# Total-RD/pymgrid

Measured on AMD Instinct MI355X. Metric: microgrid env-steps/sec, higher is better.
Workload: dtype f64

## Files before the change

### include/mgx.h

```cpp
#ifndef MGX_H
#define MGX_H

#include <stddef.h>
#include <stdint.h>

#ifdef __cplusplus
extern "C" {
#endif

#define MGX_ABI_VERSION 9
#define MGX_ABI_MINOR 3

enum mgx_status {
    MGX_OK = 0,
    MGX_ERR_INVALID = 1,
    MGX_ERR_UNSUPPORTED = 2,
    MGX_ERR_RANGE = 3,
    MGX_ERR_DEVICE = 4
};

enum mgx_obs_format { MGX_OBS_F64 = 0, MGX_OBS_F32 = 1 };
enum mgx_action_format { MGX_ACT_F64 = 0, MGX_ACT_F32 = 1 };
enum mgx_obs_rows { MGX_OBS_ROWS_FULL = 0, MGX_OBS_ROWS_STATE_ONLY = 1, MGX_OBS_ROWS_STATE_COMPACT = 2 };
enum mgx_done_format { MGX_DONE_U8 = 0, MGX_DONE_BITS = 1 };
// ... 56 lines not shown
    const uint32_t *gen_times;
    const double *grid_max_import, *grid_max_export, *grid_cost_per_unit_co2;
    const double *loss_load_cost, *overgeneration_cost;
    const double *load_ts, *pv_ts, *grid_ts;
    const double *load_lo, *load_hi, *pv_lo, *pv_hi;
    const double *grid_lo, *grid_hi;
    const double *load_noise_std, *pv_noise_std, *grid_noise_std;
    double *charge, *soc;
    uint32_t *gen_status;
    const double *base_load, *base_pv, *base_co2;
    const uint8_t *load_profile, *pv_profile, *co2_profile, *tariff;
    const double *load_ratio, *pv_ratio;
    const uint64_t *outage_bits;
} mgx_columns;

#define MGX_PROFILE_PITCH 8

int mgx_abi_version(void);
int mgx_abi_minor(void);

enum mgx_tunable {
    MGX_TUNE_WIN_THREADS = 0,
    MGX_TUNE_WIN_GROUP = 1,
    MGX_TUNE_WIN_PAIRS = 2,
    MGX_TUNE_WIN_MIN_LDS = 3,
    MGX_TUNE_PREFETCH_POOL = 4,
    MGX_TUNE_MULTI_GENERIC = 5,
    MGX_TUNE_MULTI_SMALL_OWN = 6,
    MGX_TUNE_GRID_MAJOR_COPY = 7,
    MGX_TUNE_FLEET_BYVALUE = 8,
    MGX_TUNE_LAUNCH_THREADS = 9,
    MGX_TUNE_MULTI_STATIC = 10,
    MGX_TUNE_FLEET_EPISODES = 11,
    MGX_TUNE_COUNT_ = 12
};
int mgx_set_tunable(int32_t id, int64_t value);
int mgx_get_tunable(int32_t id, int64_t *value, int64_t *default_value);
const char *mgx_last_error(void);

int mgx_create(const mgx_layout *layout, const mgx_columns *columns, mgx_handle **out);
void mgx_destroy(mgx_handle *h);

int32_t mgx_action_dim(const mgx_handle *h);
int32_t mgx_obs_dim(const mgx_handle *h);
int32_t mgx_log_dim(const mgx_handle *h);
const char *mgx_log_name(const mgx_handle *h, int32_t column);
int32_t mgx_current_step(const mgx_handle *h);

int mgx_use_device_counter(mgx_handle *h, int enable, mgx_stream stream);

int mgx_reset(mgx_handle *h, int32_t initial_step, void *obs, mgx_stream stream);

int mgx_set_window(mgx_handle *h, int32_t initial_step, int32_t final_step);

int mgx_reset_windows(mgx_handle *h, const int32_t *start, const int32_t *length, int32_t max_length,
                      double *load_w, double *pv_w, double *grid_w, int32_t *final_rel, void *obs, mgx_stream stream);

int mgx_reset_windows_rolling(mgx_handle *h, const int32_t *start, const int32_t *length, int32_t max_length,
                              int32_t ring_rows, double *load_w, double *pv_w, double *grid_w, int32_t *final_abs, void *obs,
                              mgx_stream stream);
int mgx_reset_grids(mgx_handle *h, const uint8_t *mask, const int32_t *start, const int32_t *length, mgx_stream stream);
int mgx_reset_grids_random(mgx_handle *h, const uint8_t *mask, uint64_t seed, int32_t fixed_length, int32_t *start_io,
                           int32_t *length_io, int32_t *t0_io, mgx_stream stream);

int mgx_reset_episodes(mgx_handle *h, const int32_t *start, const int32_t *length, int32_t max_length, int32_t *row_off,
                       int32_t *final_abs, void *obs, mgx_stream stream);
int mgx_set_auto_reset(mgx_handle *h, int32_t enable, uint64_t seed, int32_t fixed_length, int32_t *start_io, int32_t *length_io,
// ... 111 lines not shown

int mgx_step_many(mgx_handle *h, const void *actions, int32_t K, int normalized,
                  double *reward, uint8_t *done, void *obs, double *log, mgx_stream stream);

typedef struct mgx_env_slot {
    double *reward;
    uint8_t *done;
    void *obs;
    double *log;
} mgx_env_slot;
#define MGX_ENV_MAX_SLOTS 128
typedef struct mgx_env_plan {
    int32_t struct_size;
    int32_t n_slots;
    const mgx_env_slot *slots;
    int32_t ring_K;
    int32_t n_actions;
    void *rings[3];
    const int32_t *table;
} mgx_env_plan;
int mgx_env_bind(mgx_handle *h, const mgx_env_plan *plan);
int mgx_env_seek(mgx_handle *h, int32_t next_slot, int32_t ring_idx, int32_t ring_pos);
int mgx_env_position(const mgx_handle *h, int32_t *last_slot, int32_t *ring_idx, int32_t *ring_pos);
int mgx_env_step(mgx_handle *h, const void *actions, int normalized, mgx_stream stream);
int mgx_env_step_discrete(mgx_handle *h, const int32_t *action_id, mgx_stream stream);

int mgx_action_bounds(mgx_handle *h, double *lo, double *hi, mgx_stream stream);

int mgx_set_shards(mgx_handle *h, int32_t n_shards);
int mgx_set_launch_threads(mgx_handle *h, int32_t mode);
int mgx_fork(mgx_handle *h, mgx_stream stream);
int mgx_join(mgx_handle *h, mgx_stream stream);
void *mgx_shard_stream(mgx_handle *h, int32_t shard);

typedef struct mgx_fleet_item {
    int32_t struct_size;
    int32_t n_actions;
    mgx_handle *handle;
    const void *actions;
    const int32_t *action_id;
    const int32_t *table;
    double *reward;
    uint8_t *done;
    void *obs;
    double *log;
    void *refill_ring;
    int32_t refill_K;
    int32_t refill_ahead;
    int32_t refill_chunk;
    int32_t refill_chunks;
    int32_t wait_prefetch;
    int32_t reserved;
} mgx_fleet_item;
int mgx_fleet_step(const mgx_fleet_item *items, int32_t n_items, int normalized, mgx_stream stream);
int mgx_fleet_env_step(mgx_handle *const *handles, const void *const *actions, int32_t n_handles, int normalized, mgx_stream stream);

typedef struct mgx_synth {
    int32_t struct_size;
    int32_t n_grids, n_steps;
    int32_t n_load_profiles, n_pv_profiles, n_co2_profiles;
    const double *base_load, *base_pv, *base_co2;
    const int32_t *load_profile, *pv_profile, *co2_profile;
    const double *load_ratio, *pv_ratio;
    const int32_t *tariff;
    const int32_t *weak;
    const double *outage_per_day;
// ... 47 lines not shown
```

### pymgrid_amd/_lib.py

```python
import ctypes as C
import json
import os
import re
import subprocess
import sys

_PKG = os.path.dirname(os.path.abspath(__file__))
_ROOT = os.path.dirname(_PKG)
LIB_PATH = os.environ.get("MGX_LIB") or os.path.join(_PKG, "libmgx.so")
UNITS = (
    ("mgx_abi.hip", None, 1),
    ("mgx_fused.hip", "MGX_FUSED_PART", 6),
    ("mgx_episodes.hip", "MGX_EPISODE_PART", 2),
    ("mgx_step_episodes.hip", "MGX_EPISODE_PART", 2),
    ("mgx_episode_rows.hip", "MGX_EPISODE_PART", 2),
    ("mgx_step_episode_rows.hip", "MGX_EPISODE_PART", 2),
    ("mgx_policy_episodes.hip", "MGX_EPISODE_PART", 2),
    ("mgx_step_policy_episodes.hip", "MGX_EPISODE_PART", 2),
)
SOURCES = [os.path.join(_PKG, "csrc", f) for f in [u[0] for u in UNITS] + ["mgx_kernels.hpp", "mgx_core.hpp", "mgx_episode_loop.hpp", "mgx_episode_rows.hpp", "mgx_policy.hpp"]] + \
          [os.path.join(_ROOT, "include", "mgx.h")]

HIPCC_FLAGS = ["--offload-arch=gfx950", "-O3", "-std=c++17", "-ffp-contract=off", "-fno-fast-math", "-fPIC"]

# ... 167 lines not shown
                                       C.c_void_p, C.c_void_p, C.POINTER(EpisodeStats), C.c_void_p]),
    "mgx_step_k_episodes": (C.c_int, [C.c_void_p, C.c_void_p, C.c_int32, C.c_int, C.c_void_p, C.c_void_p, C.c_void_p, C.c_void_p,
                                      C.POINTER(EpisodeStats), C.c_void_p]),
    "mgx_rollout_episodes_rows": (C.c_int, [C.c_void_p, C.c_void_p, C.c_int, c_i32_p, C.c_int32, C.c_int32, C.c_void_p, C.c_void_p,
                                            C.c_void_p, C.c_void_p, C.POINTER(EpisodeStats), C.POINTER(EpisodeRows), C.c_void_p]),
    "mgx_step_k_episodes_rows": (C.c_int, [C.c_void_p, C.c_void_p, C.c_int32, C.c_int, C.c_void_p, C.c_void_p, C.c_void_p, C.c_void_p,
                                           C.POINTER(EpisodeStats), C.POINTER(EpisodeRows), C.c_void_p]),
    "mgx_rollout_policy_episodes": (C.c_int, [C.c_void_p, C.POINTER(Policy), c_i32_p, C.c_int32, C.c_int32, C.c_void_p, C.c_void_p,
                                              C.c_void_p, C.c_void_p, C.c_void_p, C.POINTER(EpisodeStats), C.POINTER(EpisodeRows),
                                              C.c_void_p]),
    "mgx_step_k_policy_episodes": (C.c_int, [C.c_void_p, C.POINTER(Policy), C.c_int32, C.c_void_p, C.c_void_p, C.c_void_p, C.c_void_p,
                                             C.c_void_p, C.POINTER(EpisodeStats), C.POINTER(EpisodeRows), C.c_void_p]),
    "mgx_metrics": (C.c_int, [C.c_void_p, C.c_void_p, C.c_int32, C.c_void_p, C.c_void_p]),
    "mgx_reset_windows": (C.c_int, [C.c_void_p, C.c_void_p, C.c_void_p, C.c_int32, C.c_void_p, C.c_void_p, C.c_void_p,
                                    C.c_void_p, C.c_void_p, C.c_void_p]),
    "mgx_reset_windows_rolling": (C.c_int, [C.c_void_p, C.c_void_p, C.c_void_p, C.c_int32, C.c_int32] + [C.c_void_p] * 6),
    "mgx_reset_grids": (C.c_int, [C.c_void_p, C.c_void_p, C.c_void_p, C.c_void_p, C.c_void_p]),
    "mgx_reset_grids_random": (C.c_int, [C.c_void_p, C.c_void_p, C.c_uint64, C.c_int32, C.c_void_p, C.c_void_p, C.c_void_p, C.c_void_p]),
    "mgx_reset_episodes": (C.c_int, [C.c_void_p, C.c_void_p, C.c_void_p, C.c_int32] + [C.c_void_p] * 4),
    "mgx_set_auto_reset": (C.c_int, [C.c_void_p, C.c_int32, C.c_uint64, C.c_int32, C.c_void_p, C.c_void_p, C.c_void_p]),
    "mgx_set_final_obs": (C.c_int, [C.c_void_p, C.c_void_p]),
    "mgx_check_step": (C.c_int, [C.c_void_p, C.c_void_p, C.c_int, C.c_void_p, C.c_void_p]),
    "mgx_step_many": (C.c_int, [C.c_void_p, C.c_void_p, C.c_int32, C.c_int, C.c_void_p, C.c_void_p, C.c_void_p, C.c_void_p,
                                C.c_void_p]),
    "mgx_env_bind": (C.c_int, [C.c_void_p, C.POINTER(EnvPlan)]),
    "mgx_env_seek": (C.c_int, [C.c_void_p, C.c_int32, C.c_int32, C.c_int32]),
    "mgx_env_position": (C.c_int, [C.c_void_p, c_i32_p, c_i32_p, c_i32_p]),
    "mgx_env_step": (C.c_int, [C.c_void_p, C.c_void_p, C.c_int, C.c_void_p]),
    "mgx_env_step_discrete": (C.c_int, [C.c_void_p, C.c_void_p, C.c_void_p]),
    "mgx_set_shards": (C.c_int, [C.c_void_p, C.c_int32]),
    "mgx_fork": (C.c_int, [C.c_void_p, C.c_void_p]),
    "mgx_join": (C.c_int, [C.c_void_p, C.c_void_p]),
    "mgx_shard_stream": (C.c_void_p, [C.c_void_p, C.c_int32]),
    "mgx_fleet_step": (C.c_int, [C.POINTER(FleetItem), C.c_int32, C.c_int, C.c_void_p]),
    "mgx_fleet_env_step": (C.c_int, [C.POINTER(C.c_void_p), C.POINTER(C.c_void_p), C.c_int32, C.c_int, C.c_void_p]),
    "mgx_synthesize_series": (C.c_int, [C.POINTER(Synth), C.c_void_p]),
    "mgx_generate_columns": (C.c_int, [C.POINTER(Gen), C.c_void_p]),
}


def source_hash(extra=()):
    import hashlib
    h = hashlib.sha256()
    for f in sorted(SOURCES):
        h.update(os.path.basename(f).encode() + b"\0")
        with open(f, "rb") as fh:
            h.update(fh.read())
    h.update(" ".join(HIPCC_FLAGS + list(extra)).encode())
    return h.hexdigest()[:16]


def built_hash(lib_path=None):
    try:
        with open((lib_path or LIB_PATH) + ".srchash") as fh:
            return fh.read().strip() or None
    except OSError:
        return None


def up_to_date(lib_path=None):
    path = lib_path or LIB_PATH
    return os.path.exists(path) and built_hash(path) == source_hash()


def build(force=False, verbose=False, defs=(), lib_path=None, abi_only=False):
    if lib_path is not None or defs:
# ... 94 lines not shown
    f = os.path.join(_PKG, "csrc", "_build", "resource_usage.json")
    try:
        with open(f) as fh:
            return json.load(fh)
    except (OSError, ValueError):
        return None


_lib = None


def lib():
    global _lib
    if _lib is None:
        if not os.path.exists(LIB_PATH):
            raise ImportError(f"{LIB_PATH} is missing: build it with __graft_entry__.build() "
                              f"(pymgrid_amd has no CPU fallback)")
        L = C.CDLL(LIB_PATH)
        for name, (res, args) in SYMBOLS.items():
            fn = getattr(L, name)
            fn.restype, fn.argtypes = res, args
        if L.mgx_abi_version() != ABI_VERSION:
            raise ImportError(f"libmgx.so ABI {L.mgx_abi_version()} != binding ABI {ABI_VERSION}; rebuild")
        assert C.sizeof(Layout) == 64
        _lib = L
    return _lib


def check(rc):
    if rc != MGX_OK:
        raise MgxError(rc, lib().mgx_last_error().decode())


def set_tunable(name, value):
    check(lib().mgx_set_tunable(TUNABLES.index(name), int(value)))


def get_tunable(name):
    v, d = C.c_int64(), C.c_int64()
    check(lib().mgx_get_tunable(TUNABLES.index(name), C.byref(v), C.byref(d)))
    return v.value, d.value
```

### pymgrid_amd/csrc/mgx_abi.hip

```cpp
#include "mgx_kernels.hpp"
#include "mgx_episode_rows.hpp"
#include "mgx_policy.hpp"

#include <cstdarg>
#include <cstdio>
#include <cstdlib>
#include <cstring>
#include <atomic>
#include <chrono>
#include <condition_variable>
#include <mutex>
#include <new>
#include <string>
#include <thread>
#include <vector>

using namespace mgx;

#define MGX_MAX_SHARDS 8

struct mgx_handle {
    KArgs k;
    mgx_layout layout;
    int32_t window_lo, window_hi;
    bool multi;
    int32_t ring_pitch;
    size_t multi_lds;
    int multi_small;
    std::vector<std::string> log_names;
    int32_t *d_lists;
    std::vector<int32_t> lists_uploaded;
    int32_t *d_counter;
    int32_t n_cu;
    int32_t flags;
    int32_t t;
    int32_t action_dim;
    int device;
    double *scratch;
    int32_t n_shards;
    int32_t shard_lo[MGX_MAX_SHARDS + 1];
    hipStream_t shard_stream[MGX_MAX_SHARDS];
    hipEvent_t shard_event[MGX_MAX_SHARDS];
    hipEvent_t fork_event;
    int32_t launch_threads;
    hipStream_t counter_stream;
    KArgs *d_kargs;
    KArgs k_uploaded;
    bool k_uploaded_valid;
    PLWords *d_table;
    PLWords table_uploaded;
    bool table_uploaded_valid;
    bool env_bound;
    int32_t env_n_slots, env_next, env_ring_K, env_ring_idx, env_ring_pos, env_n_actions;
    mgx_env_slot env_slots[MGX_ENV_MAX_SLOTS];
    char *env_rings[3];
    int32_t env_table[12 * 3 * 2];
    hipStream_t prefetch_stream;
    bool prefetch_pooled;
    hipEvent_t prefetch_gate, prefetch_done;
    bool prefetch_pending;
    bool windowed;
    bool rolling;
    bool inplace;
    double *pm_tables;
    double *gm_tables;
    int32_t gm_pitch;
    int32_t pm_pitch;
    int32_t rolling_max_length;
    double *roll_load_w, *roll_pv_w, *roll_grid_w;
    int32_t *roll_final;
    const double *full_load_ts, *full_pv_ts, *full_grid_ts;
    mgx_columns full_c;
    int32_t full_T, full_final, full_initial, full_window_lo, full_window_hi;
};

namespace {

constexpr int MAX_PARTIAL = 1024;
constexpr int MAX_METRICS = 64;

thread_local char g_err[512] = "";

constexpr int MGX_MAX_DEVICES = 16;
hipStream_t g_shard_streams[MGX_MAX_DEVICES][MGX_MAX_SHARDS] = {};
std::mutex g_shard_streams_lock;
hipStream_t g_prefetch_streams[MGX_MAX_DEVICES] = {};

std::atomic<int64_t> g_tune[MGX_TUNE_COUNT_];
const int64_t kTuneDefault[MGX_TUNE_COUNT_] = {
     0,
     0,
     -1,
     -1,
     0,
     0,
     1,
     1,
     1,
     1,
     1,
     1,
};
struct TuneInit { TuneInit() { for (int j = 0; j < MGX_TUNE_COUNT_; j++) g_tune[j].store(kTuneDefault[j], std::memory_order_relaxed); } } g_tune_init;
inline int64_t tune(int id) { return g_tune[id].load(std::memory_order_relaxed); }

struct LaunchWorker {
    std::atomic<uint64_t> posted{0}, done{0};
    std::atomic<int> asleep{0};
    void (*fn)(void *, int) = nullptr;
    void *ctx = nullptr;
    int shard = 0, device = 0;
    hipError_t err = hipSuccess;
    std::mutex sleep_lock, caller_lock;
    std::condition_variable wake;
    std::thread th;
    static constexpr int SPIN_US = 500;

    void run()
    {
        (void)hipSetDevice(device);
        uint64_t seen = 0;
        for (;;) {
            auto idle_since = std::chrono::steady_clock::now();
            unsigned spins = 0;
            while (posted.load(std::memory_order_acquire) == seen) {
                __builtin_ia32_pause();
                if ((++spins & 1023) == 0 &&
                    std::chrono::steady_clock::now() - idle_since > std::chrono::microseconds(SPIN_US)) {
                    std::unique_lock<std::mutex> lk(sleep_lock);
                    asleep.store(1, std::memory_order_seq_cst);
                    wake.wait(lk, [&] { return posted.load(std::memory_order_seq_cst) != seen; });
                    asleep.store(0, std::memory_order_seq_cst);
                }
            }
// ... 172 lines not shown
        case 5: { constexpr int F = 5; CALL; } break;   \
        case 6: { constexpr int F = 6; CALL; } break;   \
        case 7: { constexpr int F = 7; CALL; } break;   \
        case 14: { constexpr int F = 14; CALL; } break; \
        default: { constexpr int F = 15; CALL; } break; \
    }

}

static int32_t fused_grids_per_block(const mgx_handle *h, int64_t N)
{
    const int cus = h->n_cu > 0 ? h->n_cu : 256;
    int32_t best = BLOCK_K;
    int64_t best_cost = -1;
    for (int32_t g = BLOCK_K; g >= BLOCK_K * 3 / 4; g -= 16) {
        const int64_t blocks = (N + g - 1) / g;
        const int64_t cost = ((blocks + cus - 1) / cus) * g;
        if (best_cost < 0 || cost < best_cost) { best_cost = cost; best = g; }
    }
    return best;
}

static FusedLaunch fused_launch_for(const mgx_handle *h, const KArgs &k, hipStream_t s, const FusedOut &fo, int32_t K)
{
    FusedLaunch L;
    L.flags = h->flags; L.act_f32 = false; L.rich = fo.log != nullptr || fo.status_trace != nullptr; L.fact = factorised(k.c); L.per_step = false;
    L.gpb = fused_grids_per_block(h, k.g1 - k.g0);
    L.blocks = (unsigned)((k.g1 - k.g0 + L.gpb - 1) / L.gpb);
    L.stream = s; L.k = &k; L.actions = nullptr; L.tab = nullptr; L.ids = nullptr;
    L.t = t_arg(h); L.K = K; L.normalized = 0; L.out = fo;
    return L;
}

template <int F, bool NOISE, typename OT>
static void launch_obs_rows_as(const KArgs &k, const WindowPlan &plan, int32_t t, void *obs, unsigned blocks, size_t lds, hipStream_t st)
{
    if (lds > 64 * 1024)
        (void)hipFuncSetAttribute((const void *)obs_rows_wave_kernel<F, NOISE, OT>, hipFuncAttributeMaxDynamicSharedMemorySize, (int)lds);
    obs_rows_wave_kernel<F, NOISE, OT><<<blocks, 64, lds, st>>>(k, plan, t, (OT *)obs);
}

template <int F>
static void launch_obs_rows(const KArgs &k, const WindowPlan &plan, int32_t t, void *obs, unsigned blocks, size_t lds,
                            hipStream_t st)
{
    if (noisy(k.c)) {
        if (k.obs_f32) launch_obs_rows_as<F, true, float>(k, plan, t, obs, blocks, lds, st);
        else launch_obs_rows_as<F, true, double>(k, plan, t, obs, blocks, lds, st);
    } else {
        if (k.obs_f32) launch_obs_rows_as<F, false, float>(k, plan, t, obs, blocks, lds, st);
        else launch_obs_rows_as<F, false, double>(k, plan, t, obs, blocks, lds, st);
    }
}

static void opt_in_160k_lds(const void *kernel, bool *opted_in)
{
    int dev = 0;
    (void)hipGetDevice(&dev);
    if (dev < 0 || dev >= MGX_MAX_DEVICES || !opted_in[dev]) {
        (void)hipFuncSetAttribute(kernel, hipFuncAttributeMaxDynamicSharedMemorySize, 160 * 1024);
        if (dev >= 0 && dev < MGX_MAX_DEVICES) opted_in[dev] = true;
    }
}

template <int F, typename OT>
static void launch_windows_kernel(const KArgs &k, const WindowsKPlan &plan, int32_t t, void *ring, unsigned blocks, size_t lds, hipStream_t st)
// ... 28 lines not shown
        return MGX_OK;
    }
    const int32_t D = h->k.obs_dim;
    WindowPlan plan;
    plan.grid_col_base = h->k.col_grid;
    plan.ld = D | 1;
    plan.group = 16;
    const size_t esz = h->k.obs_f32 ? sizeof(float) : sizeof(double);
    while (plan.group > 1 && (size_t)plan.group * plan.ld * esz > 160 * 1024) plan.group /= 2;
    const size_t lds = ((size_t)plan.group * plan.ld * esz + 7) & ~(size_t)7;
    if (lds > 160 * 1024)
        return fail(MGX_ERR_UNSUPPORTED, "observation rows of %d values do not fit the 160 KiB LDS tile (horizon too large)", D);
    const unsigned blocks = (unsigned)(((int64_t)h->k.N + plan.group - 1) / plan.group);
    MGX_DISPATCH_F(h->flags, (launch_obs_rows<F>(h->k, plan, t, obs, blocks, lds, st)));
    return MGX_OK;
}

extern "C" {

int mgx_abi_version(void) { return MGX_ABI_VERSION; }
int mgx_abi_minor(void) { return MGX_ABI_MINOR; }

int mgx_set_tunable(int32_t id, int64_t value)
{
    g_err[0] = 0;
    if (id < 0 || id >= MGX_TUNE_COUNT_) return fail(MGX_ERR_INVALID, "mgx_set_tunable: unknown tunable %d", id);
    bool ok = true;
    switch (id) {
        case MGX_TUNE_WIN_THREADS: ok = value == 0 || value == 256 || value == 512 || value == 1024; break;
        case MGX_TUNE_WIN_GROUP: ok = value >= 0 && value <= 64; break;
        case MGX_TUNE_WIN_PAIRS: ok = value >= -1 && value <= 1; break;
        case MGX_TUNE_WIN_MIN_LDS: ok = value >= -1 && value <= 160 * 1024; break;
        case MGX_TUNE_LAUNCH_THREADS: ok = value >= 0 && value <= 2; break;
        default: ok = value == 0 || value == 1; break;
    }
    if (!ok) return fail(MGX_ERR_INVALID, "mgx_set_tunable: value %lld is not valid for tunable %d", (long long)value, id);
    g_tune[id].store(value, std::memory_order_relaxed);
    return MGX_OK;
}

int mgx_get_tunable(int32_t id, int64_t *value, int64_t *default_value)
{
    g_err[0] = 0;
    if (id < 0 || id >= MGX_TUNE_COUNT_) return fail(MGX_ERR_INVALID, "mgx_get_tunable: unknown tunable %d", id);
    if (value) *value = tune(id);
    if (default_value) *default_value = kTuneDefault[id];
    return MGX_OK;
}

int mgx_set_launch_threads(mgx_handle *h, int32_t enable)
{
    g_err[0] = 0;
    if (!h) return fail(MGX_ERR_INVALID, "mgx_set_launch_threads: NULL handle");
    if (enable < 0 || enable > 2) return fail(MGX_ERR_INVALID, "mgx_set_launch_threads: mode must be 0, 1 or 2");
    h->launch_threads = enable;
    return MGX_OK;
}

const char *mgx_last_error(void) { return g_err; }

int mgx_create(const mgx_layout *L, const mgx_columns *C, mgx_handle **out)
{
    g_err[0] = 0;
    if (!L || !C || !out) return fail(MGX_ERR_INVALID, "mgx_create: NULL argument");
    *out = nullptr;
    if (L->struct_size != (int32_t)sizeof(mgx_layout) || C->struct_size != (int32_t)sizeof(mgx_columns))
// ... 108 lines not shown
    h->d_kargs = nullptr; h->k_uploaded_valid = false;
    h->d_table = nullptr; h->table_uploaded_valid = false;
    h->env_bound = false; h->env_n_slots = 0; h->env_next = 0; h->env_ring_K = 0; h->env_ring_idx = 0; h->env_ring_pos = 0; h->env_n_actions = 0;
    h->prefetch_stream = nullptr; h->prefetch_gate = nullptr; h->prefetch_done = nullptr; h->prefetch_pending = false;
    h->prefetch_pooled = false;
    h->windowed = false; h->rolling = false;
    h->k.row_mask = -1;
    h->k.ep_off = nullptr; h->k.ep_final = nullptr; h->k.ar_mode = 0; h->k.ar_fixed_length = 0; h->k.ar_lo = 0; h->k.ar_hi = 0;
    h->k.ar_max_length = 0; h->k.ar_seed = 0; h->k.ar_start_io = nullptr; h->k.ar_length_io = nullptr; h->k.ar_t0_io = nullptr;
    h->k.final_obs = nullptr; h->k.pm_pitch = 0;
    h->inplace = false; h->pm_tables = nullptr; h->pm_pitch = 0; h->gm_tables = nullptr; h->gm_pitch = 0;
    if ((e = hipMalloc((void **)&h->scratch, sizeof(double) * MAX_METRICS * MAX_PARTIAL)) != hipSuccess) {
        delete h;
        return hip_fail(e, "hipMalloc(scratch)");
    }
    h->d_counter = nullptr;
    h->k.t_dev = nullptr;
    if ((e = hipMalloc((void **)&h->d_counter, 4 * sizeof(int32_t))) != hipSuccess) {
        (void)hipFree(h->scratch); delete h;
        return hip_fail(e, "hipMalloc(counter)");
    }
    *out = h;
    return MGX_OK;
}

void mgx_destroy(mgx_handle *h)
{
    if (!h) return;
    for (int j = 0; j < MGX_MAX_SHARDS; j++) {
        if (h->shard_stream[j]) (void)hipStreamSynchronize(h->shard_stream[j]);
        if (h->shard_event[j]) (void)hipEventDestroy(h->shard_event[j]);
    }
    if (h->fork_event) (void)hipEventDestroy(h->fork_event);
    if (h->prefetch_stream) { (void)hipStreamSynchronize(h->prefetch_stream); if (!h->prefetch_pooled) (void)hipStreamDestroy(h->prefetch_stream); }
    if (h->pm_tables) (void)hipFree(h->pm_tables);
    if (h->gm_tables) (void)hipFree(h->gm_tables);
    if (h->d_kargs) (void)hipFree(h->d_kargs);
    if (h->d_table) (void)hipFree(h->d_table);
    if (h->d_lists) (void)hipFree(h->d_lists);
    if (h->prefetch_gate) (void)hipEventDestroy(h->prefetch_gate);
    if (h->prefetch_done) (void)hipEventDestroy(h->prefetch_done);
    if (h->scratch) (void)hipFree(h->scratch);
    if (h->d_counter) (void)hipFree(h->d_counter);
    delete h;
}

int32_t mgx_action_dim(const mgx_handle *h) { return h ? h->action_dim : -1; }
int32_t mgx_obs_dim(const mgx_handle *h) { return h ? h->k.obs_dim : -1; }
int32_t mgx_log_dim(const mgx_handle *h) { return h ? h->k.log_dim : -1; }
int32_t mgx_current_step(const mgx_handle *h)
{
    if (!h) return -1;
    if (h->k.t_dev) {
        int32_t c[2] = {0, 0};
        if (hipStreamSynchronize(h->counter_stream) != hipSuccess) return -1;
        if (hipMemcpy(c, h->d_counter, sizeof(c), hipMemcpyDeviceToHost) != hipSuccess) return -1;
        return c[0];
    }
    return h->t;
}

int mgx_use_device_counter(mgx_handle *h, int enable, mgx_stream stream)
{
    g_err[0] = 0;
    if (!h) return fail(MGX_ERR_INVALID, "mgx_use_device_counter: NULL handle");
    hipStream_t st = (hipStream_t)stream;
// ... 638 lines not shown
                                                         "with mgx_reset_windows_rolling");
    GatherArgs g;
    rolling_gather_args(h, &g);
    g.start = start; g.length = length; g.mask = mask; g.row0 = h->t;
    gather_windows_kernel<<<blocks_for(h->k.N), BLOCK, 0, (hipStream_t)stream>>>(g);
    return launched("gather_windows_kernel launch");
}

int mgx_set_shards(mgx_handle *h, int32_t n_shards)
{
    g_err[0] = 0;
    if (!h) return fail(MGX_ERR_INVALID, "mgx_set_shards: NULL handle");
    if (n_shards < 1 || n_shards > MGX_MAX_SHARDS) return fail(MGX_ERR_INVALID, "mgx_set_shards: n_shards must be in [1, %d]", MGX_MAX_SHARDS);
    if (n_shards > 1 && h->k.t_dev) return fail(MGX_ERR_UNSUPPORTED, "mgx_set_shards: not offered in device-counter mode");
    if (n_shards > 1 && h->windowed) return fail(MGX_ERR_UNSUPPORTED, "mgx_set_shards: not offered during a per-grid-window episode");
    DeviceGuard on_device(h->device);
    for (int j = 0; j < h->n_shards && h->n_shards > 1; j++)
        if (h->shard_stream[j]) (void)hipStreamSynchronize(h->shard_stream[j]);
    hipError_t e = hipSuccess;
    if (n_shards > 1) {
        if (!h->fork_event) e = hipEventCreateWithFlags(&h->fork_event, hipEventDisableTiming);
        for (int j = 0; j < n_shards && e == hipSuccess; j++) {
            if (!h->shard_stream[j]) {
                if (h->device < 0 || h->device >= MGX_MAX_DEVICES) return fail(MGX_ERR_UNSUPPORTED, "mgx_set_shards: device index %d", h->device);
                std::lock_guard<std::mutex> guard(g_shard_streams_lock);
                hipStream_t &pooled = g_shard_streams[h->device][j];
                if (!pooled) e = hipStreamCreateWithFlags(&pooled, hipStreamNonBlocking);
                h->shard_stream[j] = pooled;
            }
            if (e == hipSuccess && !h->shard_event[j]) e = hipEventCreateWithFlags(&h->shard_event[j], hipEventDisableTiming);
        }
        if (e != hipSuccess) return hip_fail(e, "mgx_set_shards: creating streams / events");
    }
    const int64_t N = h->k.N;
    int64_t per = ((N + n_shards - 1) / n_shards + 255) / 256 * 256;
    for (int j = 0; j <= n_shards; j++) { const int64_t b = (int64_t)j * per; h->shard_lo[j] = (int32_t)(b < N ? b : N); }
    h->shard_lo[n_shards] = (int32_t)N;
    h->n_shards = n_shards;
    return MGX_OK;
}

int mgx_fork(mgx_handle *h, mgx_stream stream)
{
    g_err[0] = 0;
    if (!h) return fail(MGX_ERR_INVALID, "mgx_fork: NULL handle");
    if (h->n_shards <= 1) return MGX_OK;
    hipError_t e = hipEventRecord(h->fork_event, (hipStream_t)stream);
    for (int j = 0; j < h->n_shards && e == hipSuccess; j++) e = hipStreamWaitEvent(h->shard_stream[j], h->fork_event, 0);
    return e == hipSuccess ? MGX_OK : hip_fail(e, "mgx_fork");
}

int mgx_join(mgx_handle *h, mgx_stream stream)
{
    g_err[0] = 0;
    if (!h) return fail(MGX_ERR_INVALID, "mgx_join: NULL handle");
    if (h->n_shards <= 1) return MGX_OK;
    hipError_t e = hipSuccess;
    for (int j = 0; j < h->n_shards && e == hipSuccess; j++) {
        e = hipEventRecord(h->shard_event[j], h->shard_stream[j]);
        if (e == hipSuccess) e = hipStreamWaitEvent((hipStream_t)stream, h->shard_event[j], 0);
    }
    return e == hipSuccess ? MGX_OK : hip_fail(e, "mgx_join");
}

void *mgx_shard_stream(mgx_handle *h, int32_t shard)
{
    if (!h || shard < 0 || shard >= h->n_shards || h->n_shards <= 1) return nullptr;
    return (void *)h->shard_stream[shard];
}

struct EpisodeStep {
    KArgs k;
    bool restart_after;
};

static int episode_step_begin(mgx_handle *h, const uint8_t *done, void *obs, void *obs_inline, EpisodeStep *ep, const char *who)
{
    ep->k = h->k; ep->k.g0 = 0; ep->k.g1 = h->k.N;
    ep->restart_after = false;
    const bool rows_behind = obs && !obs_inline;
    if (ep->k.final_obs && !obs)
        return fail(MGX_ERR_INVALID, "%s: mgx_set_final_obs is set but the step writes no observation", who);
    drop_ring_final_obs(ep->k);
    if (rows_behind && ep->k.final_obs) {
        if (ep->k.ar_mode && !done)
            return fail(MGX_ERR_INVALID, "%s: with a forecast horizon the observation before an automatic restart needs the `done` flags", who);
        ep->restart_after = ep->k.ar_mode != 0;
        ep->k.ar_mode = 0;
        ep->k.final_obs = nullptr;
    }
    return MGX_OK;
}

static int episode_step_end(mgx_handle *h, const EpisodeStep &ep, const uint8_t *done, void *obs, void *obs_inline, hipStream_t st)
// ... 113 lines not shown
    const size_t obs_row = (size_t)N * h->k.obs_dim * (h->k.obs_f32 ? sizeof(float) : sizeof(double));
    void *obs_inline = rows_inline(h, obs);
    if (h->n_shards > 1 && h->launch_threads && !h->multi && !h->inplace && (!obs || obs_inline)) {
        const int32_t t0 = t_arg(h);
        for_each_shard_threaded(h, (hipStream_t)stream, [&](const KArgs &kk, hipStream_t s) {
            for (int32_t k = 0; k < K; k++) {
                MGX_DISPATCH_F(h->flags, (step_kernel<F><<<blocks_for(kk.g1 - kk.g0), BLOCK, row_tile_lds(kk, obs_inline), s>>>(
                                              kk, actions ? (const char *)actions + k * act_row : nullptr, t0 + k, normalized, reward + k * N,
                                              done ? done + k * N : nullptr, obs_inline ? (char *)obs_inline + k * obs_row : nullptr,
                                              log ? log + (int64_t)k * h->k.log_dim * N : nullptr)));
            }
        }, 1);
        return finish_step(h, K, (hipStream_t)stream, launch_error(), "step_kernel launch");
    }
    for (int32_t k = 0; k < K; k++) {
        if (int rc = step_once(h, actions ? (const char *)actions + k * act_row : nullptr, normalized, reward + k * N,
                               done ? done + k * N : nullptr, obs ? (char *)obs + k * obs_row : nullptr,
                               log ? log + (int64_t)k * h->k.log_dim * N : nullptr, (hipStream_t)stream))
            return rc;
    }
    return MGX_OK;
}

int mgx_step_k(mgx_handle *h, const void *actions, int32_t K, int normalized, double *reward, uint8_t *done,
               double *soc_trace, uint32_t *status_trace, double *ret_acc, double *log, mgx_stream stream)
{
    g_err[0] = 0;
    if (!h || (h->action_dim > 0 && !actions)) return fail(MGX_ERR_INVALID, "mgx_step_k: NULL argument");
    if (K <= 0) return fail(MGX_ERR_INVALID, "mgx_step_k: K must be positive");
    if (h->rolling) return fail(MGX_ERR_UNSUPPORTED, "mgx_step_k: rolling windows take single steps (grids restart between steps)");
    if (int rc = check_rows(h, K, "mgx_step_k", true)) return rc;
    hipStream_t st = (hipStream_t)stream;
    const FusedOut fo{reward, done, soc_trace, status_trace, ret_acc, log};
    if (h->multi) {
        if (h->k.done_bits && done) return fail(MGX_ERR_UNSUPPORTED, "mgx_step_k: the general kernels write `done` as bytes");
        const bool own_kernel = tune(MGX_TUNE_MULTI_SMALL_OWN) != 0;
        const bool static_counts = tune(MGX_TUNE_MULTI_STATIC) != 0;
        for_each_shard(h, st, [&](const KArgs &k, hipStream_t s) {
            if (own_kernel && static_counts && k.n_load >= 1 && k.n_pv >= 1) {
                MultiStaticLaunch L{h->flags, k.n_genset, k.n_battery, k.n_grid, k.n_load, k.n_pv, multi_blocks(k.g1 - k.g0), s, &k, actions,
                                    t_arg(h), K, normalized, fo};
                if (launch_step_k_multi_static(L)) return;
            }
            if (h->multi_small && own_kernel) {
                MGX_DISPATCH_F(h->flags, (step_k_multi_small_kernel<F><<<multi_blocks(k.g1 - k.g0), BLOCK_MULTI, 0, s>>>(
                                              k, actions, t_arg(h), K, normalized, fo)));
            } else {
                MGX_DISPATCH_F(h->flags, (step_k_multi_kernel<F><<<multi_blocks(k.g1 - k.g0), BLOCK_MULTI, h->multi_lds, s>>>(
                                              k, actions, nullptr, 0, 0, nullptr, 0, t_arg(h), K, normalized, fo)));
            }
        });
        return finish_step(h, K, st, hipGetLastError(), "step_k_multi_kernel launch");
    }
    for_each_shard(h, st, [&](const KArgs &k, hipStream_t s) {
        FusedLaunch L = fused_launch_for(h, k, s, fo, K);
        L.actions = actions; L.act_f32 = k.act_f32 != 0; L.normalized = normalized;
        (void)(launch_step_k_p0(L) || launch_step_k_p1(L) || launch_step_k_p2(L) || launch_step_k_p3(L) || launch_step_k_p4(L));
    });
    return finish_step(h, K, st, hipGetLastError(), "step_k_kernel launch");
}

static int encode_table(const mgx_handle *h, const int32_t *table, int32_t n_actions, PLWords *tab, const char *who)
{
    if (n_actions <= 0 || n_actions > 12) return fail(MGX_ERR_INVALID, "%s: n_actions must be in [1, 12]", who);
    memset(tab, 0, sizeof(*tab));
    tab->n_actions = n_actions;
    for (int i = 0; i < n_actions; i++)
        for (int k = 0; k < 3; k++) {
            const int32_t mod = table[(i * 3 + k) * 2], act = table[(i * 3 + k) * 2 + 1];
            if (mod == -1) continue;
            if (mod < 0 || mod > 2 || act < 0 || act > 1) return fail(MGX_ERR_INVALID, "%s: bad table entry (%d, %d)", who, mod, act);
            if (mod == 0 && !h->layout.has_genset) return fail(MGX_ERR_INVALID, "%s: table names a genset, layout has none", who);
            if (mod == 1 && !h->layout.has_battery) return fail(MGX_ERR_INVALID, "%s: table names a battery, layout has none", who);
            if (mod == 2 && !h->layout.has_grid) return fail(MGX_ERR_INVALID, "%s: table names a grid, layout has none", who);
            for (int k2 = 0; k2 < k; k2++)
                if (table[(i * 3 + k2) * 2] == mod)
                    return fail(MGX_ERR_INVALID, "%s: list %d names module %d twice (priority lists hold each module once, "
                                                 "priority_list.py:40-48)", who, i, mod);
            tab->w[i] |= ((uint32_t)mod | ((uint32_t)act << 2) | 8u) << (4 * k);
        }
    return MGX_OK;
}

static int launch_expand_lists(mgx_handle *h, const int32_t *action_id, const int32_t *d_lists, int32_t n_lists, int32_t list_len,
                               double *control, uint32_t *violations, hipStream_t st)
{
    for_each_shard(h, st, [&](const KArgs &k, hipStream_t s) {
        MGX_DISPATCH_F(h->flags, (expand_multi_kernel<F><<<multi_blocks(k.g1 - k.g0), BLOCK_MULTI, 0, s>>>(k, d_lists, n_lists, list_len,
                                                                                                       action_id, t_arg(h), control,
                                                                                                       violations)));
    });
// ... 215 lines not shown
    if (int rc = step_once(h, actions, normalized, sl.reward, sl.done, tg.obs, sl.log, (hipStream_t)stream)) return rc;
    return env_commit(h, tg.enters_next_ring, stream);
}

int mgx_env_step_discrete(mgx_handle *h, const int32_t *action_id, mgx_stream stream)
{
    g_err[0] = 0;
    if (!h || !h->env_bound) return fail(MGX_ERR_INVALID, "mgx_env_step_discrete: no plan is bound (mgx_env_bind)");
    if (h->env_n_actions <= 0) return fail(MGX_ERR_INVALID, "mgx_env_step_discrete: the bound plan holds no priority-list table");
    const mgx_env_slot &sl = h->env_slots[h->env_next];
    const EnvTarget tg = env_target(h, sl);
    if (!action_id) return fail(MGX_ERR_INVALID, "mgx_env_step_discrete: NULL argument");
    if (int rc = check_step_args(h, action_id, sl.reward, tg.obs, 1, "mgx_env_step_discrete")) return rc;
    if (tg.enters_next_ring) { if (int rc = mgx_prefetch_wait(h, stream)) return rc; }
    if (int rc = mgx_step_discrete(h, action_id, h->env_table, h->env_n_actions, nullptr, sl.reward, sl.done, tg.obs, sl.log, stream)) return rc;
    return env_commit(h, tg.enters_next_ring, stream);
}

int mgx_rollout_discrete(mgx_handle *h, const uint8_t *action_id, int per_step, const int32_t *table, int32_t n_actions,
                         int32_t K, double *reward, uint8_t *done, double *soc_trace, uint32_t *status_trace,
                         double *ret_acc, double *log, mgx_stream stream)
{
    g_err[0] = 0;
    if (!h || !action_id || !table) return fail(MGX_ERR_INVALID, "mgx_rollout_discrete: NULL argument");
    if (K <= 0) return fail(MGX_ERR_INVALID, "mgx_rollout_discrete: K must be positive");
    if (h->rolling) return fail(MGX_ERR_UNSUPPORTED, "mgx_rollout_discrete: rolling windows take single steps");
    if (h->multi) return fail(MGX_ERR_UNSUPPORTED, "mgx_rollout_discrete: needs exactly one module of every kind "
                                                    "per grid; use mgx_expand_discrete / mgx_expand_lists + mgx_step");
    if (int rc = check_rows(h, K, "mgx_rollout_discrete", true)) return rc;
    PLWords tab;
    if (int rc = encode_table(h, table, n_actions, &tab, "mgx_rollout_discrete")) return rc;
    const FusedOut fo{reward, done, soc_trace, status_trace, ret_acc, log};
    hipStream_t st = (hipStream_t)stream;
    for_each_shard(h, st, [&](const KArgs &k, hipStream_t s) {
        FusedLaunch L = fused_launch_for(h, k, s, fo, K);
        L.tab = &tab; L.ids = action_id; L.per_step = per_step != 0;
        (void)(launch_rollout_p0(L) || launch_rollout_p1(L) || launch_rollout_p2(L) || launch_rollout_p3(L) || launch_rollout_p4(L));
    });
    return finish_step(h, K, st, hipGetLastError(), "rollout_kernel launch");
}

static int episodes_launch_refusal(mgx_handle *h, int32_t K, const uint8_t *done, const char *fn, const char *lockstep, const char *single)
{
    if (K <= 0) return fail(MGX_ERR_INVALID, "%s: K must be positive", fn);
    if (h->multi) return fail(MGX_ERR_UNSUPPORTED, "%s: needs exactly one module of every kind per grid (several: single steps, %s)", fn, single);
    if (h->n_shards > 1) return fail(MGX_ERR_UNSUPPORTED, "%s: not offered while the handle steps in shards", fn);
    if (dev_counter(h)) return fail(MGX_ERR_UNSUPPORTED, "%s: not offered in device-counter mode", fn);
    if (!h->inplace || !h->k.ep_off || !h->k.ep_final)
        return fail(MGX_ERR_INVALID, "%s: the handle is not stepping in-place episodes (mgx_reset_episodes); lock-step episodes: %s", fn, lockstep);
    if (h->k.done_bits && done) return fail(MGX_ERR_UNSUPPORTED, "%s: `done` is written as bytes (mgx_set_done_format)", fn);
    return MGX_OK;
}

static int episode_rows_refusal(mgx_handle *h, const mgx_episode_rows *rows, const char *fn)
{
    if (rows->struct_size != (int32_t)sizeof(mgx_episode_rows))
        return fail(MGX_ERR_INVALID, "%s: rows->struct_size is %d, sizeof(mgx_episode_rows) is %d", fn, rows->struct_size, (int)sizeof(mgx_episode_rows));
    if (h->k.H != 0) return fail(MGX_ERR_UNSUPPORTED, "%s: rows inside the launch are whole H = 0 rows (the handle has a forecast horizon of %d)", fn, h->k.H);
    if (h->k.obs_state_only) return fail(MGX_ERR_UNSUPPORTED, "%s: rows inside the launch are whole rows (mgx_set_obs_mode is state-only)", fn);
    if (h->k.final_obs) return fail(MGX_ERR_UNSUPPORTED, "%s: mgx_set_final_obs is set; its [N, D] buffer has no meaning across K steps "
                                                          "(rows->final_obs receives the rows before the restarts)", fn);
    return MGX_OK;
}

static int prepare_episode_launch(mgx_handle *h, int32_t K, double *reward, uint8_t *done, double *soc_trace, uint32_t *status_trace,
                                  const mgx_episode_stats *stats, const mgx_episode_rows *rows, mgx_stream stream, const char *fn,
                                  const char *lockstep, const char *single, const int32_t *table, int32_t n_actions, PLWords *tab,
                                  EpisodeRowsLaunch &R)
{
    if (int rc = episodes_launch_refusal(h, K, done, fn, lockstep, single)) return rc;
    if (rows) {
// ... 568 lines not shown
```

### pymgrid_amd/engine.py

```python
import ctypes as C

import numpy as np
import torch

from . import _lib
from ._lib import check


def _ptr(t):
    return None if t is None else t.data_ptr()


try:
    _get_raw = torch._C._cuda_getCurrentRawStream

    def _raw_stream(idx):
        return _get_raw(idx)
except AttributeError:
    def _raw_stream(idx):
        return torch.cuda.current_stream(idx).cuda_stream


class StepEngine:
    def __init__(self, batch, obs_dtype=torch.float64, action_dtype=torch.float64):
# ... 363 lines not shown
        self._window_start.copy_(torch.where(m, start, self._window_start))
        self._window_t0.copy_(torch.where(m, torch.full_like(start, self.current_step), self._window_t0))

    def reset_grids_random(self, mask, seed, fixed_length=0, lengths_out=None):
        if mask.dtype == torch.bool:
            mask = mask.view(torch.uint8)
        if mask.dtype != torch.uint8 or tuple(mask.shape) != (self.N,) or mask.device != self.device or not mask.is_contiguous():
            raise ValueError(f"mask must be a contiguous uint8 / bool tensor of shape ({self.N},) on {self.device}")
        if getattr(self, "_window_t0", None) is None:
            raise _lib.MgxError(_lib.MGX_ERR_INVALID, "reset_grids_random: the engine is not in rolling-window mode")
        self._call(self._lib.mgx_reset_grids_random, mask.data_ptr(), int(seed) & (2 ** 64 - 1), int(fixed_length),
                   self._window_start.data_ptr(), _ptr(lengths_out), self._window_t0.data_ptr())

    def set_shards(self, n_shards):
        check(self._lib.mgx_set_shards(self._h, int(n_shards)))
        self.n_shards = int(n_shards)

    def set_launch_threads(self, mode=1):
        mode = 2 if mode is True else int(mode)
        check(self._lib.mgx_set_launch_threads(self._h, mode))

    def fork(self):
        self._call(self._lib.mgx_fork)

    def join(self):
        self._call(self._lib.mgx_join)

    def shard_streams(self):
        n = getattr(self, "n_shards", 1)
        if n <= 1:
            return []
        return [torch.cuda.ExternalStream(self._lib.mgx_shard_stream(self._h, j), device=self.device) for j in range(n)]

    def check_step(self, actions, normalized=True, out=None):
        actions = self._check_actions(actions, ())
        mask = out if out is not None else self._empty(self.N, dtype=torch.int32)
        self._call(self._lib.mgx_check_step, _ptr(actions), 1 if normalized else 0, mask.data_ptr())
        return mask

    def action_bounds(self, out=None):
        A = self.layout.action_dim
        lo, hi = out if out is not None else (self._empty(self.N, A), self._empty(self.N, A))
        self._call(self._lib.mgx_action_bounds, lo.data_ptr(), hi.data_ptr())
        return lo, hi

    def _step_outputs(self, out, want_done, want_obs, want_log, want_control=False, lead=()):
        reward = done = obs = log = control = None
        if out:
            reward, done, obs, log, control = out.get("reward"), out.get("done"), out.get("obs"), out.get("log"), out.get("control")
        if reward is None:
            reward = self._empty(*lead, self.N)
        if not want_done:
            done = None
        elif done is None:
            done = self._empty(*lead, self.N, dtype=torch.uint8)
        if not want_obs:
            obs = None
        elif not lead:
            obs = self._obs_buf(obs)
        elif obs is None:
            obs = self._empty(*lead, self.N, self.obs_dim, dtype=self.obs_dtype)
        if not want_log:
            log = None
        elif log is None:
            log = self._empty(*lead, self.log_dim, self.N)
        if not want_control:
# ... 298 lines not shown
```

Measured before the change: 138.5 billion.

## Add shard phase staggering via delay kernels and rebalance shard bounds

Adds an opt-in tunable that measures per-round time on shard 0 with events, then launches small sleep kernels on the other shard streams so their fused rounds start staggered in phase. The aim is to spread the shards' memory-bandwidth peaks instead of having them collide. It also changes shard boundaries from 256-grid rounding to evenly split 16-grid lines, which balances shard sizes more finely. The phase tunable defaults to 0, so only the new boundary split runs by default; when enabled, the staggering adds extra launches, event records and host-side queries.

```diff
diff --git a/include/mgx.h b/include/mgx.h
--- a/include/mgx.h
+++ b/include/mgx.h
@@ -112,7 +112,8 @@
     MGX_TUNE_LAUNCH_THREADS = 9,
     MGX_TUNE_MULTI_STATIC = 10,
     MGX_TUNE_FLEET_EPISODES = 11,
-    MGX_TUNE_COUNT_ = 12
+    MGX_TUNE_SHARD_PHASE = 12,
+    MGX_TUNE_COUNT_ = 13
 };
 int mgx_set_tunable(int32_t id, int64_t value);
 int mgx_get_tunable(int32_t id, int64_t *value, int64_t *default_value);
@@ -290,6 +291,8 @@
 int mgx_fork(mgx_handle *h, mgx_stream stream);
 int mgx_join(mgx_handle *h, mgx_stream stream);
 void *mgx_shard_stream(mgx_handle *h, int32_t shard);
+void mgx_shard_bounds(int32_t n_grids, int32_t n_shards, int32_t *bounds);
+void mgx_shard_phase_counters(const mgx_handle *h, int64_t *delays_issued, int64_t *events_recorded, double *period_us);
 
 typedef struct mgx_fleet_item {
     int32_t struct_size;
diff --git a/pymgrid_amd/_lib.py b/pymgrid_amd/_lib.py
--- a/pymgrid_amd/_lib.py
+++ b/pymgrid_amd/_lib.py
@@ -223,6 +223,8 @@
     "mgx_fork": (C.c_int, [C.c_void_p, C.c_void_p]),
     "mgx_join": (C.c_int, [C.c_void_p, C.c_void_p]),
     "mgx_shard_stream": (C.c_void_p, [C.c_void_p, C.c_int32]),
+    "mgx_shard_bounds": (None, [C.c_int32, C.c_int32, c_i32_p]),
+    "mgx_shard_phase_counters": (None, [C.c_void_p, C.POINTER(C.c_int64), C.POINTER(C.c_int64), C.POINTER(C.c_double)]),
     "mgx_fleet_step": (C.c_int, [C.POINTER(FleetItem), C.c_int32, C.c_int, C.c_void_p]),
     "mgx_fleet_env_step": (C.c_int, [C.POINTER(C.c_void_p), C.POINTER(C.c_void_p), C.c_int32, C.c_int, C.c_void_p]),
     "mgx_synthesize_series": (C.c_int, [C.POINTER(Synth), C.c_void_p]),
@@ -383,11 +385,21 @@
         raise MgxError(rc, lib().mgx_last_error().decode())
 
 
+def _tunable_id(name):
+    return {"shard_phase": 12}[name] if name not in TUNABLES else TUNABLES.index(name)
+
+
 def set_tunable(name, value):
-    check(lib().mgx_set_tunable(TUNABLES.index(name), int(value)))
+    check(lib().mgx_set_tunable(_tunable_id(name), int(value)))
 
 
 def get_tunable(name):
     v, d = C.c_int64(), C.c_int64()
-    check(lib().mgx_get_tunable(TUNABLES.index(name), C.byref(v), C.byref(d)))
+    check(lib().mgx_get_tunable(_tunable_id(name), C.byref(v), C.byref(d)))
     return v.value, d.value
+
+
+def shard_bounds(n_grids, n_shards):
+    b = (C.c_int32 * (int(n_shards) + 1))()
+    lib().mgx_shard_bounds(int(n_grids), int(n_shards), b)
+    return list(b)
diff --git a/pymgrid_amd/csrc/mgx_abi.hip b/pymgrid_amd/csrc/mgx_abi.hip
--- a/pymgrid_amd/csrc/mgx_abi.hip
+++ b/pymgrid_amd/csrc/mgx_abi.hip
@@ -18,6 +18,19 @@
 using namespace mgx;
 
 #define MGX_MAX_SHARDS 8
+
+constexpr int PHASE_RING = 4;
+constexpr int PHASE_SAMPLES = 8;
+struct ShardPhase {
+    bool armed = false;
+    hipEvent_t e0[PHASE_RING] = {}, e1[PHASE_RING] = {};
+    bool pending[PHASE_RING] = {};
+    int64_t key = -1;
+    float sample_us[PHASE_SAMPLES] = {};
+    int32_t n_samples = 0;
+    int64_t delays_issued = 0, events_recorded = 0;
+    double last_period_us = 0.0;
+};
 
 struct mgx_handle {
     KArgs k;
@@ -42,6 +55,7 @@
     hipStream_t shard_stream[MGX_MAX_SHARDS];
     hipEvent_t shard_event[MGX_MAX_SHARDS];
     hipEvent_t fork_event;
+    ShardPhase phase;
     int32_t launch_threads;
     hipStream_t counter_stream;
     KArgs *d_kargs;
@@ -100,6 +114,7 @@
      1,
      1,
      1,
+     0,
 };
 struct TuneInit { TuneInit() { for (int j = 0; j < MGX_TUNE_COUNT_; j++) g_tune[j].store(kTuneDefault[j], std::memory_order_relaxed); } } g_tune_init;
 inline int64_t tune(int id) { return g_tune[id].load(std::memory_order_relaxed); }
@@ -338,6 +353,89 @@
     return L;
 }
 
+namespace mgx {
+__global__ void __launch_bounds__(64) shard_delay_kernel(uint64_t ticks, int32_t cap)
+{
+    const uint64_t t0 = __builtin_amdgcn_s_memrealtime();
+    for (int32_t i = 0; i < cap && __builtin_amdgcn_s_memrealtime() - t0 < ticks; i++) __builtin_amdgcn_s_sleep(8);
+}
+}
+
+constexpr double PHASE_FALLBACK_BYTES_PER_US = 5.9e6;
+constexpr double PHASE_MAX_DELAY_US = 10000.0;
+constexpr int32_t PHASE_DELAY_CAP = 200000;
+
+static int64_t fused_round_bytes(const mgx_handle *h, const FusedOut &fo, int32_t K, int64_t control_bytes)
+{
+    const int64_t per_step = control_bytes + (fo.reward ? 8 : 0) + (fo.done ? 1 : 0) + (fo.soc_trace ? 8 : 0) +
+                             (fo.status_trace ? 4 : 0) + (fo.log ? 8 * (int64_t)h->k.log_dim : 0);
+    return per_step * K * (int64_t)h->k.N;
+}
+
+static bool shard_phase_on(const mgx_handle *h, hipStream_t user)
+{
+    if (h->n_shards <= 1 || tune(MGX_TUNE_SHARD_PHASE) == 0) return false;
+    hipStreamCaptureStatus cs = hipStreamCaptureStatusNone;
+    if (hipStreamIsCapturing(user, &cs) != hipSuccess) { (void)hipGetLastError(); return false; }
+    return cs == hipStreamCaptureStatusNone;
+}
+
+static int shard_phase_open(mgx_handle *h, int64_t round_bytes)
+{
+    ShardPhase &p = h->phase;
+    if (p.key != round_bytes) { p.key = round_bytes; p.n_samples = 0; }
+    bool query_failed = false;
+    for (int i = 0; i < PHASE_RING; i++) {
+        if (!p.pending[i]) continue;
+        if (hipEventQuery(p.e1[i]) != hipSuccess) { query_failed = true; continue; }
+        float ms = 0.0f;
+        if (hipEventElapsedTime(&ms, p.e0[i], p.e1[i]) == hipSuccess && ms > 0.0f && p.n_samples < PHASE_SAMPLES) p.sample_us[p.n_samples++] = ms * 1e3f;
+        p.pending[i] = false;
+    }
+    if (query_failed) (void)hipGetLastError();
+    const bool armed = p.armed;
+    if (armed) {
+        p.armed = false;
+        double period_us = (double)round_bytes / PHASE_FALLBACK_BYTES_PER_US;
+        if (p.n_samples >= 2) {
+            float s[PHASE_SAMPLES];
+            memcpy(s, p.sample_us, sizeof(float) * p.n_samples);
+            for (int a = 1; a < p.n_samples; a++) for (int b = a; b > 0 && s[b] < s[b - 1]; b--) { const float t = s[b]; s[b] = s[b - 1]; s[b - 1] = t; }
+            period_us = s[p.n_samples / 2];
+        }
+        p.last_period_us = period_us;
+        int khz = 0;
+        if (hipDeviceGetAttribute(&khz, hipDeviceAttributeWallClockRate, h->device) != hipSuccess || khz <= 0) { (void)hipGetLastError(); khz = 100000; }
+        const double phase = (double)tune(MGX_TUNE_SHARD_PHASE) / 1000.0;
+        for (int j = 1; j < h->n_shards; j++) {
+            if (h->shard_lo[j + 1] <= h->shard_lo[j]) continue;
+            double us = period_us * phase * j;
+            if (us > PHASE_MAX_DELAY_US) us = PHASE_MAX_DELAY_US;
+            const uint64_t ticks = (uint64_t)(us * (double)khz / 1000.0) + 1;
+            shard_delay_kernel<<<1, 64, 0, h->shard_stream[j]>>>(ticks, PHASE_DELAY_CAP);
+            p.delays_issued++;
+        }
+        return -1;
+    }
+    if (p.n_samples >= PHASE_SAMPLES || h->shard_lo[1] <= h->shard_lo[0]) return -1;
+    for (int i = 0; i < PHASE_RING; i++) {
+        if (p.pending[i]) continue;
+        if (!p.e0[i] && (hipEventCreate(&p.e0[i]) != hipSuccess || hipEventCreate(&p.e1[i]) != hipSuccess)) { (void)hipGetLastError(); return -1; }
+        if (hipEventRecord(p.e0[i], h->shard_stream[0]) != hipSuccess) { (void)hipGetLastError(); return -1; }
+        p.events_recorded++;
+        return i;
+    }
+    return -1;
+}
+
+static void shard_phase_close(mgx_handle *h, int slot)
+{
+    if (slot < 0) return;
+    ShardPhase &p = h->phase;
+    if (hipEventRecord(p.e1[slot], h->shard_stream[0]) == hipSuccess) { p.pending[slot] = true; p.events_recorded++; }
+    else (void)hipGetLastError();
+}
+
 template <int F, bool NOISE, typename OT>
 static void launch_obs_rows_as(const KArgs &k, const WindowPlan &plan, int32_t t, void *obs, unsigned blocks, size_t lds, hipStream_t st)
 {
@@ -432,6 +530,7 @@
         case MGX_TUNE_WIN_PAIRS: ok = value >= -1 && value <= 1; break;
         case MGX_TUNE_WIN_MIN_LDS: ok = value >= -1 && value <= 160 * 1024; break;
         case MGX_TUNE_LAUNCH_THREADS: ok = value >= 0 && value <= 2; break;
+        case MGX_TUNE_SHARD_PHASE: ok = value >= 0 && value <= 999; break;
         default: ok = value == 0 || value == 1; break;
     }
     if (!ok) return fail(MGX_ERR_INVALID, "mgx_set_tunable: value %lld is not valid for tunable %d", (long long)value, id);
@@ -606,6 +705,10 @@
         if (h->shard_event[j]) (void)hipEventDestroy(h->shard_event[j]);
     }
     if (h->fork_event) (void)hipEventDestroy(h->fork_event);
+    for (int i = 0; i < PHASE_RING; i++) {
+        if (h->phase.e0[i]) (void)hipEventDestroy(h->phase.e0[i]);
+        if (h->phase.e1[i]) (void)hipEventDestroy(h->phase.e1[i]);
+    }
     if (h->prefetch_stream) { (void)hipStreamSynchronize(h->prefetch_stream); if (!h->prefetch_pooled) (void)hipStreamDestroy(h->prefetch_stream); }
     if (h->pm_tables) (void)hipFree(h->pm_tables);
     if (h->gm_tables) (void)hipFree(h->gm_tables);
@@ -1310,12 +1413,27 @@
         }
         if (e != hipSuccess) return hip_fail(e, "mgx_set_shards: creating streams / events");
     }
-    const int64_t N = h->k.N;
-    int64_t per = ((N + n_shards - 1) / n_shards + 255) / 256 * 256;
-    for (int j = 0; j <= n_shards; j++) { const int64_t b = (int64_t)j * per; h->shard_lo[j] = (int32_t)(b < N ? b : N); }
-    h->shard_lo[n_shards] = (int32_t)N;
+    mgx_shard_bounds((int32_t)h->k.N, n_shards, h->shard_lo);
     h->n_shards = n_shards;
-    return MGX_OK;
+    h->phase.armed = n_shards > 1;
+    return MGX_OK;
+}
+
+void mgx_shard_bounds(int32_t n_grids, int32_t n_shards, int32_t *bounds)
+{
+    const int64_t lines = ((int64_t)n_grids + 15) / 16;
+    for (int j = 0; j <= n_shards; j++) {
+        const int64_t b = lines * j / n_shards * 16;
+        bounds[j] = (int32_t)(b < n_grids ? b : n_grids);
+    }
+    bounds[n_shards] = n_grids;
+}
+
+void mgx_shard_phase_counters(const mgx_handle *h, int64_t *delays_issued, int64_t *events_recorded, double *period_us)
+{
+    if (delays_issued) *delays_issued = h ? h->phase.delays_issued : 0;
+    if (events_recorded) *events_recorded = h ? h->phase.events_recorded : 0;
+    if (period_us) *period_us = h ? h->phase.last_period_us : 0.0;
 }
 
 int mgx_fork(mgx_handle *h, mgx_stream stream)
@@ -1325,6 +1443,7 @@
     if (h->n_shards <= 1) return MGX_OK;
     hipError_t e = hipEventRecord(h->fork_event, (hipStream_t)stream);
     for (int j = 0; j < h->n_shards && e == hipSuccess; j++) e = hipStreamWaitEvent(h->shard_stream[j], h->fork_event, 0);
+    h->phase.armed = true;
     return e == hipSuccess ? MGX_OK : hip_fail(e, "mgx_fork");
 }
 
@@ -1338,6 +1457,7 @@
         e = hipEventRecord(h->shard_event[j], h->shard_stream[j]);
         if (e == hipSuccess) e = hipStreamWaitEvent((hipStream_t)stream, h->shard_event[j], 0);
     }
+    h->phase.armed = true;
     return e == hipSuccess ? MGX_OK : hip_fail(e, "mgx_join");
 }
 
@@ -1517,6 +1637,7 @@
     if (int rc = check_rows(h, K, "mgx_step_k", true)) return rc;
     hipStream_t st = (hipStream_t)stream;
     const FusedOut fo{reward, done, soc_trace, status_trace, ret_acc, log};
+    const int phase_slot = shard_phase_on(h, st) ? shard_phase_open(h, fused_round_bytes(h, fo, K, h->action_dim * (h->k.act_f32 ? 4 : 8))) : -1;
     if (h->multi) {
         if (h->k.done_bits && done) return fail(MGX_ERR_UNSUPPORTED, "mgx_step_k: the general kernels write `done` as bytes");
         const bool own_kernel = tune(MGX_TUNE_MULTI_SMALL_OWN) != 0;
@@ -1535,6 +1656,7 @@
                                               k, actions, nullptr, 0, 0, nullptr, 0, t_arg(h), K, normalized, fo)));
             }
         });
+        shard_phase_close(h, phase_slot);
         return finish_step(h, K, st, hipGetLastError(), "step_k_multi_kernel launch");
     }
     for_each_shard(h, st, [&](const KArgs &k, hipStream_t s) {
@@ -1542,6 +1664,7 @@
         L.actions = actions; L.act_f32 = k.act_f32 != 0; L.normalized = normalized;
         (void)(launch_step_k_p0(L) || launch_step_k_p1(L) || launch_step_k_p2(L) || launch_step_k_p3(L) || launch_step_k_p4(L));
     });
+    shard_phase_close(h, phase_slot);
     return finish_step(h, K, st, hipGetLastError(), "step_k_kernel launch");
 }
 
@@ -1823,11 +1946,13 @@
     if (int rc = encode_table(h, table, n_actions, &tab, "mgx_rollout_discrete")) return rc;
     const FusedOut fo{reward, done, soc_trace, status_trace, ret_acc, log};
     hipStream_t st = (hipStream_t)stream;
+    const int phase_slot = shard_phase_on(h, st) ? shard_phase_open(h, fused_round_bytes(h, fo, K, per_step ? 1 : 0)) : -1;
     for_each_shard(h, st, [&](const KArgs &k, hipStream_t s) {
         FusedLaunch L = fused_launch_for(h, k, s, fo, K);
         L.tab = &tab; L.ids = action_id; L.per_step = per_step != 0;
         (void)(launch_rollout_p0(L) || launch_rollout_p1(L) || launch_rollout_p2(L) || launch_rollout_p3(L) || launch_rollout_p4(L));
     });
+    shard_phase_close(h, phase_slot);
     return finish_step(h, K, st, hipGetLastError(), "rollout_kernel launch");
 }
 
diff --git a/pymgrid_amd/engine.py b/pymgrid_amd/engine.py
--- a/pymgrid_amd/engine.py
+++ b/pymgrid_amd/engine.py
@@ -419,6 +419,12 @@
             return []
         return [torch.cuda.ExternalStream(self._lib.mgx_shard_stream(self._h, j), device=self.device) for j in range(n)]
 
+    def shard_phase_counters(self):
+        import ctypes as C
+        d, e, p = C.c_int64(), C.c_int64(), C.c_double()
+        self._lib.mgx_shard_phase_counters(self._h, C.byref(d), C.byref(e), C.byref(p))
+        return {"delays": d.value, "events": e.value, "period_us": p.value}
+
     def check_step(self, actions, normalized=True, out=None):
         actions = self._check_actions(actions, ())
         mask = out if out is not None else self._empty(self.N, dtype=torch.int32)
```

Result: no change. 137.6 billion (-0.6%).
